# steineggerlab/Metabuli

Hardware: AMD Instinct MI355X
Metric: Mreads/s classified (metabuli classify hot path, reads + index resident in HBM) (higher is better)
Workload: dtype u64

## Files before the change

metabuli_amd/csrc/kernels_extract.h:

```cpp
#ifndef MTB_KERNELS_EXTRACT_H
#define MTB_KERNELS_EXTRACT_H
#include "dev_util.h"
#include "mtb_core.h"

#define MTB_EXTRACT_STAGE 320

struct ExtractArgs {
    const char *bases; const uint64_t *offs;
    const char *bases2; const uint64_t *offs2;
    uint64_t n_reads;
    int32_t seq_mode, syncmer, smer_len, kmer_format;
    int32_t tag_ord;
    int32_t dig_shift;
};

#define MTB_EXTRACT_BUF 320
#define MTB_EXTRACT_CHUNK 8192
template <int MODE>
__global__ __launch_bounds__(64) void k_extract(ExtractArgs a, const mtb_tables *__restrict__ tabs,
                                                uint32_t *__restrict__ counts, const uint64_t *__restrict__ out_offs,
                                                mtb_kmer *__restrict__ out, int32_t *__restrict__ qlen,
                                                int32_t *__restrict__ qlen2, uint32_t *__restrict__ max_len,
                                                unsigned long long *__restrict__ counter, uint64_t out_cap,
                                                uint16_t *__restrict__ dig_out = nullptr, uint8_t *__restrict__ off_flags = nullptr) {
    constexpr bool EMIT = MODE != 0;
    constexpr bool STATS = MODE != 1;
    __shared__ mtb_kmer s_out[MODE == 2 ? MTB_EXTRACT_BUF : 1];
    __shared__ unsigned long long s_base;
    uint32_t n_buf = 0;
    uint64_t chunk_pos = 0, chunk_end = 0, produced = 0, reads_done = 0, cur_read = 0;
    bool overflow = false;
    auto flush = [&]() {
        if (MODE != 2 || n_buf == 0) return;
        __syncthreads();
        uint32_t done = 0;
        while (done < n_buf) {
            if (chunk_pos == chunk_end) {
                const uint64_t need = n_buf - done;
                const uint64_t rem_reads = (a.n_reads - 1 - cur_read) / gridDim.x + 1;
                const uint64_t avg = reads_done ? produced / reads_done + 1 : 128;
                uint64_t size = need + rem_reads * avg * 5 / 4 + 64;
                size = size < MTB_EXTRACT_CHUNK ? size : MTB_EXTRACT_CHUNK;
                size = size < need ? need : size;
                if (threadIdx.x == 0) s_base = atomicAdd(counter, (unsigned long long)size);
                __syncthreads();
                chunk_pos = (uint64_t)s_base; chunk_end = chunk_pos + size;
                __syncthreads();
                if (chunk_end > out_cap) { overflow = true; chunk_pos = chunk_end; break; }
            }
            const uint32_t room = (uint32_t)(chunk_end - chunk_pos < (uint64_t)(n_buf - done) ? chunk_end - chunk_pos : (uint64_t)(n_buf - done));
            for (uint32_t i = threadIdx.x; i < room; i += 64) {
                const mtb_kmer x = s_out[done + i];
                out[chunk_pos + i] = x;
                if (dig_out) {
                    uint32_t two = (uint32_t)(x.value >> a.dig_shift) & 1023u, d = (two >> 5) * 21u + (two & 31u);
                    dig_out[chunk_pos + i] = (uint16_t)(d < 511u ? d : 511u);
                }
            }
            chunk_pos += room; done += room;
        }
        produced += n_buf;
        __syncthreads();
        n_buf = 0;
    };
    __shared__ mtb_tables s_tab;
    __shared__ __attribute__((aligned(8))) uint8_t s_cod[80];
    __shared__ __attribute__((aligned(8))) uint8_t s_cod3[MODE == 2 ? 3 : 1][MODE == 2 ? 120 : 8];
    __shared__ uint8_t s_code[MTB_EXTRACT_STAGE];
    const uint32_t lane = threadIdx.x;
    for (uint32_t i = lane; i < sizeof(mtb_tables) / 4; i += 64) ((uint32_t *)&s_tab)[i] = ((const uint32_t *)tabs)[i];
    __syncthreads();
    uint32_t my_max = 0, my_maxq = 0;
    uint32_t el_max = 0, el_maxq = 0, n_off = 0;
    const bool paired = a.seq_mode == 2;
    for (uint64_t r = blockIdx.x; r < a.n_reads; r += gridDim.x) {
        cur_read = r; reads_done++;
        const uint64_t o1 = a.offs[r];
        const int32_t len1 = (int32_t)(a.offs[r + 1] - o1);
        uint64_t o2 = 0; int32_t len2 = 0;
        if (paired) { o2 = a.offs2[r]; len2 = (int32_t)(a.offs2[r + 1] - o2); }
        const int32_t ql1 = mtb_used_len(len1), ql2 = paired ? mtb_used_len(len2) : 0;
        if (STATS) {
            if (lane == 0) { qlen[r] = ql1; qlen2[r] = ql2; }
            uint32_t tot_len = (uint32_t)(ql1 + ql2);
            my_max = tot_len > my_max ? tot_len : my_max;
        }
        const bool skip = mtb_read_too_short(len1) || (paired && mtb_read_too_short(len2));
        if (skip) { if ((MODE == 0 || (MODE == 2 && counts)) && lane == 0) counts[r] = 0; continue; }
        uint64_t wpos = MODE == 1 ? out_offs[r] : 0;
        uint32_t total = 0;
        for (int mate = 0; mate < (paired ? 2 : 1); mate++) {
            const char *seq = mate ? a.bases2 + o2 : a.bases + o1;
            const int32_t len = mate ? len2 : len1;
            const uint32_t pos_off = mate ? (uint32_t)(ql1 + 3) : 0u;
            const int32_t used = mtb_used_len(len);
            const int32_t n_cod = used / 3, n_win = n_cod - 7;
            const bool old_fmt = a.kmer_format == 1;
            const bool staged = !old_fmt && len <= MTB_EXTRACT_STAGE;
            if (staged) {
                __syncthreads();
                for (int32_t i = (int32_t)lane; i < len; i += 64) s_code[i] = s_tab.base[(uint8_t)seq[i]];
                __syncthreads();
            }
            if (MODE == 2 && staged) {
                for (int strand = 0; strand < 2; strand++) {
                    const bool fwd = strand == 0;
                    const bool back = !fwd;
                    __syncthreads();
                    for (int fi = 0; fi < 3; fi++) {
                        const int32_t begin = mtb_frame_begin(len, strand * 3 + fi);
                        for (int32_t j = (int32_t)lane; j < n_cod; j += 64)
                            s_cod3[fi][j] = mtb_codon_byte_codes(&s_tab, s_code, mtb_codon_ci(begin, used, j, fwd), fwd);
                    }
                    __syncthreads();
                    const int32_t n_all = 3 * n_win;
                    for (int32_t c0 = 0; c0 < n_all; c0 += 64) {
                        const int32_t cidx = c0 + (int32_t)lane;
                        const int32_t fi = (cidx >= n_win) + (cidx >= 2 * n_win);
                        const int32_t wi = cidx - fi * n_win;
                        const int32_t w = back ? n_win - 1 - wi : wi;
                        bool ok = false; uint64_t v = 0;
                        if (cidx < n_all) {
                            const uint32_t *c32 = (const uint32_t *)&s_cod3[fi][0];
                            const uint32_t q = (uint32_t)w >> 2, sh = (uint32_t)w & 3u;
                            const uint32_t x0 = c32[q], x1 = c32[q + 1], x2 = c32[q + 2];
                            ok = mtb_window_metamer_words(__builtin_amdgcn_alignbyte(x1, x0, sh), __builtin_amdgcn_alignbyte(x2, x1, sh), a.syncmer, a.smer_len, &v);
                        }
                        const uint64_t mask = __ballot(ok);
                        const uint32_t c = (uint32_t)__popcll(mask);
                        if (n_buf + c > MTB_EXTRACT_BUF) flush();
                        if (ok) {
                            const int f = strand * 3 + fi;
                            const int32_t begin = mtb_frame_begin(len, f);
                            const uint32_t below = (uint32_t)__popcll(mask & lanemask_lt());
                            uint32_t pf = mtb_window_pos(begin, used, w, fwd) + pos_off;
                            if (a.tag_ord) { const uint32_t ord = total + below; pf |= (ord < 0xFFFFu ? ord : 0xFFFFu) << 16; }
                            mtb_kmer k; k.value = v; k.qinfo = mtb_qinfo((uint32_t)(r + 1), pf, (uint32_t)f);
                            s_out[n_buf + below] = k;
                        }
                        n_buf += c; total += c;
                    }
                }
            } else
            for (int f = 0; f < 6; f++) {
                const bool fwd = f < 3;
                const int32_t begin = mtb_frame_begin(len, f);
                const bool back = MODE == 2 && a.tag_ord && (old_fmt ? fwd : !fwd);
                const int32_t n_chunk = (n_win + 63) / 64;
                for (int32_t cw = 0; cw < n_chunk; cw++) {
                    const int32_t w0 = (back ? n_chunk - 1 - cw : cw) * 64;
                    int32_t j = w0 + (int32_t)lane;
                    int32_t j2 = w0 + 64 + (int32_t)lane;
                    if (staged) {
                        if (j < n_cod) s_cod[lane] = mtb_codon_byte_codes(&s_tab, s_code, mtb_codon_ci(begin, used, j, fwd), fwd);
                        if (lane < 8 && j2 < n_cod) s_cod[64 + lane] = mtb_codon_byte_codes(&s_tab, s_code, mtb_codon_ci(begin, used, j2, fwd), fwd);
                    } else if (old_fmt) {
                        if (j < n_cod) s_cod[lane] = mtb_codon_byte_old(&s_tab, seq, mtb_codon_ci_old(begin, used, j, fwd), fwd);
                        if (lane < 8 && j2 < n_cod) s_cod[64 + lane] = mtb_codon_byte_old(&s_tab, seq, mtb_codon_ci_old(begin, used, j2, fwd), fwd);
                    } else {
                        if (j < n_cod) s_cod[lane] = mtb_codon_byte(&s_tab, seq, mtb_codon_ci(begin, used, j, fwd), fwd);
                        if (lane < 8 && j2 < n_cod) s_cod[64 + lane] = mtb_codon_byte(&s_tab, seq, mtb_codon_ci(begin, used, j2, fwd), fwd);
                    }
                    __syncthreads();
                    int32_t w = w0 + (int32_t)lane;
                    bool ok = false; uint64_t v = 0;
                    if (w < n_win) {
                        if (old_fmt) ok = mtb_window_metamer_old(&s_cod[lane], &v);
                        else {
                            const uint32_t *c32 = (const uint32_t *)s_cod;
                            const uint32_t q = lane >> 2, sh = lane & 3u;
                            const uint32_t x0 = c32[q], x1 = c32[q + 1], x2 = c32[q + 2];
                            ok = mtb_window_metamer_words(__builtin_amdgcn_alignbyte(x1, x0, sh), __builtin_amdgcn_alignbyte(x2, x1, sh), a.syncmer, a.smer_len, &v);
                        }
                    }
                    uint64_t mask = __ballot(ok);
                    uint32_t c = (uint32_t)__popcll(mask);
// ... 43 lines not shown
```

metabuli_amd/csrc/kernels_score_fast.h:

```cpp
#ifndef MTB_KERNELS_SCORE_FAST_H
#define MTB_KERNELS_SCORE_FAST_H
#include "dev_util.h"
#include "kernels_score.h"
#include "mtb_core.h"
#include "mtb_score_par.h"

#define MTB_FAST_BKT 128
#ifndef MTB_FAST_MERGE_SINGLES
#define MTB_FAST_MERGE_SINGLES 0
#endif

#ifdef MTB_FAST_DEBUG
__device__ unsigned long long mtb_fast_reasons[32];
#define MTB_FAST_COUNT(k, v) do { if (threadIdx.x == 0) atomicAdd(&mtb_fast_reasons[k], (unsigned long long)(v)); } while (0)
#define MTB_FAST_T0() unsigned long long ft_ = __builtin_readcyclecounter()
#define MTB_FAST_MARK(k) do { const unsigned long long t_ = __builtin_readcyclecounter(); if (threadIdx.x == 0) s_ph[k] += t_ - ft_; ft_ = t_; } while (0)
#else
#define MTB_FAST_COUNT(k, v) do {} while (0)
#define MTB_FAST_T0() do {} while (0)
#define MTB_FAST_MARK(k) do {} while (0)
#endif

#define MTB_DPP_RED(v, OP) do { \
    { const uint32_t o_ = (uint32_t)__builtin_amdgcn_update_dpp((int)(v), (int)(v), 0x111, 0xF, 0xF, false); (v) = OP((v), o_); } \
    { const uint32_t o_ = (uint32_t)__builtin_amdgcn_update_dpp((int)(v), (int)(v), 0x112, 0xF, 0xF, false); (v) = OP((v), o_); } \
    { const uint32_t o_ = (uint32_t)__builtin_amdgcn_update_dpp((int)(v), (int)(v), 0x114, 0xF, 0xF, false); (v) = OP((v), o_); } \
    { const uint32_t o_ = (uint32_t)__builtin_amdgcn_update_dpp((int)(v), (int)(v), 0x118, 0xF, 0xF, false); (v) = OP((v), o_); } \
    { const uint32_t o_ = (uint32_t)__builtin_amdgcn_update_dpp((int)(v), (int)(v), 0x142, 0xA, 0xF, false); (v) = OP((v), o_); } \
    { const uint32_t o_ = (uint32_t)__builtin_amdgcn_update_dpp((int)(v), (int)(v), 0x143, 0xC, 0xF, false); (v) = OP((v), o_); } } while (0)
#define MTB_MINU(a, b) ((b) < (a) ? (b) : (a))
#define MTB_MAXU(a, b) ((b) > (a) ? (b) : (a))
__device__ __forceinline__ uint32_t wave_min_u32(uint32_t v) { MTB_DPP_RED(v, MTB_MINU); return (uint32_t)__builtin_amdgcn_readlane((int)v, 63); }
__device__ __forceinline__ uint32_t wave_max_u32(uint32_t v) { MTB_DPP_RED(v, MTB_MAXU); return (uint32_t)__builtin_amdgcn_readlane((int)v, 63); }

struct FKey { uint32_t lo, hi; };
__device__ __forceinline__ uint32_t fk_species(const FKey &k) { return k.hi >> 10; }
__device__ __forceinline__ uint32_t fk_frame(const FKey &k) { return (k.hi >> 7) & 7u; }
__device__ __forceinline__ uint32_t fk_pos(const FKey &k) { return ((k.hi & 127u) << 4) | (k.lo >> 27); }
__device__ __forceinline__ uint32_t fk_ham(const FKey &k) { return (k.lo >> 24) & 7u; }
__device__ __forceinline__ uint32_t fk_dna(const FKey &k) { return k.lo & 0xFFFFFFu; }

struct FastPath { int32_t start, end; float score; int32_t ham; uint32_t rehs;  int32_t species; };

template <int K, int KL = K, bool BYFRAME = false>
__global__ __launch_bounds__(64, K <= 3 ? 5 : 4) void k_score_fast(const mtb_slot16 *__restrict__ slots_all, uint64_t n_reads, const int32_t *__restrict__ qlen,
                                                       const int32_t *__restrict__ qlen2, mtb_tax_view tx, mtb_score_params sp,
                                                       const uint64_t *__restrict__ tc_off, mtb_result *__restrict__ results,
                                                       int32_t *__restrict__ tc_tax, uint32_t *__restrict__ tc_cnt, uint64_t tc_cap, uint64_t tc_base,
                                                       const uint32_t *__restrict__ cursor, uint32_t stride, uint32_t direct, uint32_t epoch,
                                                       uint8_t *__restrict__ slow_flag, uint32_t *__restrict__ cnt_out) {
    constexpr int NMAX = 64 * K;
    __shared__ FKey s_key[NMAX];
    __shared__ uint64_t s_aux[NMAX];
    __shared__ uint64_t s_pp[NMAX];
    __shared__ FastPath s_path[64];
    __shared__ uint32_t s_pf[64];
    __shared__ uint32_t s_tl[(BYFRAME || MTB_FAST_MERGE_SINGLES) ? 64 : 1];
    typedef uint32_t __attribute__((may_alias)) u32a; typedef int32_t __attribute__((may_alias)) i32a;
    static_assert(NMAX * 8 >= 2 * MTB_FAST_BKT * 4 && NMAX * 8 >= 256 * 4 && NMAX * 8 >= (MTB_LR_MAXE + MTB_LR_MAXE * MTB_LR_K) * 4, "tables fit the arrays they live in");
    u32a *const s_hcnt = (u32a *)s_pp;
    u32a *const s_hmin = (u32a *)s_key; i32a *const s_btax = (i32a *)s_key + MTB_FAST_BKT;
    i32a *const s_otax = (i32a *)s_pp; u32a *const s_ocnt = (u32a *)s_pp + MTB_FAST_BKT;
    i32a *const s_lev = (i32a *)s_aux; i32a *const s_anc = (i32a *)s_aux + MTB_LR_MAXE;
    const int32_t lane = (int32_t)threadIdx.x;
    MTB_BEGIN_ACQUIRE();
#ifdef MTB_FAST_DEBUG
    __shared__ unsigned long long s_ph[16];
    if (threadIdx.x < 16) s_ph[threadIdx.x] = 0;
#endif
    const uint64_t lt = lanemask_lt();
    const uint64_t le = lt | (1ull << lane);
    const uint32_t tail_cap = stride - direct;
    const uint32_t div_m = (65536u + (uint32_t)sp.dna_shift - 1u) / (uint32_t)sp.dna_shift;
    const uint32_t lines = (stride * (uint32_t)sizeof(mtb_slot16) + 127u) / 128u;

    for (uint64_t r = blockIdx.x; r < n_reads; r += gridDim.x) {
        if (r + gridDim.x < n_reads && (uint32_t)lane < lines) {
            const uint8_t *pf = (const uint8_t *)(slots_all + (r + gridDim.x) * (uint64_t)stride) + (uint64_t)lane * 128u;
            __builtin_amdgcn_global_load_lds((const __attribute__((address_space(1))) void *)pf, (__attribute__((address_space(3))) void *)s_pf, 4, 0, 0);
        }
        MTB_FAST_T0();
        const int32_t ql1 = qlen[r], ql2 = qlen2[r];
        const int32_t read_len = ql1 + ql2;
        const int32_t nb = mtb_num_buckets(read_len, sp.dna_shift);
        const uint32_t cur = cursor[r];
        const mtb_slot16 *slots = slots_all + r * (uint64_t)stride;
        mtb_slot16 x[KL];
#pragma unroll
        for (int k = 0; k < KL; k++) { const uint32_t i = (uint32_t)lane + 64u * k; x[k].a = 0; x[k].b = 0; if (i < stride) x[k] = slots[i]; }
        bool slow = cur > tail_cap || nb > MTB_FAST_BKT;
        wave_fence();
        MTB_FAST_MARK(0);
        int32_t n = 0, n_live = 0;
        uint32_t spc[KL]; bool live[KL]; int32_t dst[KL];
        uint32_t smin = 0xFFFFFFFFu, smax = 0u;
#pragma unroll
        for (int k = 0; k < KL; k++) {
            const uint32_t i = (uint32_t)lane + 64u * k;
            live[k] = i < stride && mtb_slot_epoch(x[k]) == epoch && (i < direct || i - direct < cur);
            spc[k] = live[k] ? (uint32_t)(x[k].a >> 32) : 0xFFFFFFFFu;
            dst[k] = 0;
            n_live += (int32_t)__popcll(__ballot(live[k]));
            smin = spc[k] < smin ? spc[k] : smin;
            if (live[k]) smax = spc[k] > smax ? spc[k] : smax;
        }
        smin = wave_min_u32(smin); smax = wave_max_u32(smax);
        uint32_t todo_min = 0xFFFFFFFFu;
        if (smin != smax) {
            for (int32_t q = lane; q < 256; q += 64) s_hcnt[q] = 0;
            wave_fence();
#pragma unroll
            for (int k = 0; k < KL; k++) if (live[k]) atomicAdd(&s_hcnt[(spc[k] * 0x9E3779B1u) >> 24], 1u);
            wave_fence();
#pragma unroll
            for (int k = 0; k < KL; k++) if (live[k] && s_hcnt[(spc[k] * 0x9E3779B1u) >> 24] < 2u) { live[k] = false; spc[k] = 0xFFFFFFFFu; }
        } else if (n_live < 2) {
#pragma unroll
            for (int k = 0; k < KL; k++) { live[k] = false; spc[k] = 0xFFFFFFFFu; }
        }
        if (BYFRAME) {
#pragma unroll
            for (int k = 0; k < KL; k++) if (live[k]) spc[k] = (spc[k] << 3) | ((uint32_t)(x[k].b >> 52) & 7u);
        }
#pragma unroll
        for (int k = 0; k < KL; k++) todo_min = spc[k] < todo_min ? spc[k] : todo_min;
        for (int round = 0; ; round++) {
            const uint32_t m = wave_min_u32(todo_min);
            if (m == 0xFFFFFFFFu) break;
            if (round == 24) { slow = true; break; }
            todo_min = 0xFFFFFFFFu;
#pragma unroll
            for (int k = 0; k < KL; k++) {
                const bool mine = spc[k] == m;
                const uint64_t mask = __ballot(mine);
                if (mine) { dst[k] = n + (int32_t)__popcll(mask & lt); spc[k] = 0xFFFFFFFFu; }
                n += (int32_t)__popcll(mask);
                todo_min = spc[k] < todo_min ? spc[k] : todo_min;
            }
        }
        if (KL > K && n > NMAX) slow = true;
#pragma unroll
        for (int k = 0; k < KL; k++) {
            if (live[k] && !slow) {
                const uint64_t b = x[k].b;
                const uint32_t bh = (uint32_t)(b >> 32), ps_ = (bh >> 8) & 0x7FFu;
                FKey fk; fk.hi = ((uint32_t)(x[k].a >> 32) << 10) | (((bh >> 20) & 7u) << 7) | (ps_ >> 4);
                fk.lo = ((ps_ & 15u) << 27) | (((bh >> 23) & 7u) << 24) | ((uint32_t)b & 0xFFFFFFu);
                s_key[dst[k]] = fk;
                s_aux[dst[k]] = (x[k].a & 0xFFFFFFFFull) | (((b >> 24) & 0xFFFFull) << 32) | ((uint32_t)lane + 64u * k >= direct ? (1ull << 63) : 0ull);
            }
        }
        MTB_FAST_MARK(1);
        mtb_result R = mtb_result_blank(ql1, ql2, (uint32_t)tc_base);
        if (!slow && n == 0) { if (lane == 0) { cnt_out[r] = (uint32_t)n_live; results[r] = R; } continue; }
        wave_fence();
        {
            uint32_t nt = 0;
            bool any_tail = false;
#pragma unroll
            for (int k = 0; k < KL; k++) any_tail |= live[k] && (uint32_t)lane + 64u * k >= direct;
            if ((BYFRAME || MTB_FAST_MERGE_SINGLES) && !slow && __any(any_tail)) {
                FKey ke[K]; uint64_t ax[K]; int32_t np[K]; bool tl[K];
                const int32_t nsl = (n + 63) >> 6;
#pragma unroll
                for (int k = 0; k < K; k++) {
                    const int32_t i = lane + 64 * k;
                    ke[k].lo = 0; ke[k].hi = 0; ax[k] = 0; np[k] = i; tl[k] = false;
                    if (k < nsl && i < n) { ke[k] = s_key[i]; ax[k] = s_aux[i]; tl[k] = (ax[k] >> 63) != 0; }
                    if (k < nsl) {
                        const uint64_t tm = __ballot(tl[k]);
                        if (tl[k]) { const uint32_t at = nt + (uint32_t)__popcll(tm & lt); if (at < 64u) s_tl[at] = (uint32_t)i; }
                        nt += (uint32_t)__popcll(tm);
                    }
                }
                if (nt > 64u) slow = true;
                wave_fence();
                if (!slow) {
                    auto same_run = [&](const FKey &a, const FKey &b) { return BYFRAME ? ((a.hi ^ b.hi) >> 7) == 0 : ((a.hi ^ b.hi) >> 10) == 0; };
                    auto less = [&](const FKey &a, const FKey &b) { return a.hi < b.hi || (a.hi == b.hi && a.lo < b.lo); };
                    for (uint32_t t = 0; t < nt; t++) {
                        const int32_t ti = (int32_t)s_tl[t];
                        const FKey kt = s_key[ti];
                        uint32_t n_dir_less = 0, n_dir_run = 0;
#pragma unroll
                        for (int k = 0; k < K; k++) {
                            if (k < nsl) {
                                const int32_t i = lane + 64 * k;
                                const bool dir = i < n && !tl[k] && same_run(ke[k], kt);
                                const bool smaller = dir && less(ke[k], kt);
                                if (dir && !smaller) np[k]++;
                                n_dir_run += (uint32_t)__popcll(__ballot(dir)); n_dir_less += (uint32_t)__popcll(__ballot(smaller));
                            }
                        }
                        uint32_t n_tl_less = 0, n_tl_before = 0;
                        for (uint32_t u = 0; u < nt; u++) {
                            if (u == t) continue;
                            const FKey ku = s_key[s_tl[u]];
                            if (!same_run(ku, kt)) continue;
                            n_tl_less += (less(ku, kt) || (!less(kt, ku) && u < t)) ? 1u : 0u; n_tl_before += u < t ? 1u : 0u;
                        }
                        const int32_t run_start = ti - (int32_t)n_dir_run - (int32_t)n_tl_before;
#pragma unroll
                        for (int k = 0; k < K; k++) if (lane + 64 * k == ti) np[k] = run_start + (int32_t)(n_dir_less + n_tl_less);
                    }
                    wave_fence();
#pragma unroll
                    for (int k = 0; k < K; k++) { const int32_t i = lane + 64 * k; if (k < nsl && i < n) { s_key[np[k]] = ke[k]; s_aux[np[k]] = ax[k] & ~(1ull << 63); } }
                    wave_fence();
                }
            }
        }
        FKey key[K]; uint32_t tid[K], reh[K];
        int32_t tcanon[K]; uint8_t euk[K];
        const mtb_tax_node *nodes = (const mtb_tax_node *)tx.node;
        bool bhead[K], linked[K];
        int32_t shv[K];
        uint64_t bmask[K + 1], lmask[K + 1], rmask[K];
        const int32_t nslot = (n + 63) >> 6;
        bool bad = false, bad2 = false;
#ifdef MTB_FAST_DEBUG
        if (slow) MTB_FAST_COUNT(cur > tail_cap || nb > MTB_FAST_BKT ? 0 : 1, 1);
#endif
#pragma unroll
        for (int k = 0; k < K; k++) {
            const int32_t i = lane + 64 * k;
            key[k].lo = 0; key[k].hi = 0; tid[k] = 0; reh[k] = 0; bhead[k] = true; linked[k] = false; shv[k] = 0; tcanon[k] = -1; euk[k] = 0;
            bmask[k] = ~0ull; lmask[k] = 0; rmask[k] = 0;
            if (k < nslot && !slow) {
                FKey pk; pk.lo = 0; pk.hi = 0;
                if (i < n) {
                    key[k] = s_key[i]; const uint64_t a = s_aux[i]; tid[k] = (uint32_t)a; reh[k] = (uint32_t)(a >> 32) & 0xFFFFu; if (i > 0) pk = s_key[i - 1];
                }
                {
                    const int32_t t_ = (int32_t)tid[k], s_ = (int32_t)fk_species(key[k]);
                    const bool tv = i < n && t_ >= 0 && t_ <= tx.max_taxid, sv = i < n && s_ >= 0 && s_ <= tx.max_taxid;
                    const int32_t tc_ = nodes[tv ? t_ : 0].canon; const uint8_t eu_ = tx.under_euk[sv ? s_ : 0];
                    tcanon[k] = tv ? tc_ : -1; euk[k] = sv ? eu_ : 0;
                }
                const bool first = i == 0;
                if (i < n && !first) {
                    if (pk.hi > key[k].hi || (pk.hi == key[k].hi && pk.lo > key[k].lo)) bad = true;
                    if (pk.hi == key[k].hi && ((pk.lo ^ key[k].lo) >> 27) == 0) bad2 = true;
                }
                bhead[k] = i >= n || first || ((pk.hi ^ key[k].hi) >> 7) != 0;
                if (i < n && !bhead[k]) {
                    const int32_t pos = (int32_t)fk_pos(key[k]), ppos = (int32_t)fk_pos(pk);
                    const int32_t s = (pos - ppos) / 3;
                    if (s > 0 && s <= sp.max_codon_shift) {
                        shv[k] = s;
                        const bool fwd = fk_frame(key[k]) < 3u;
                        linked[k] = mtb_consecutive(fk_dna(pk), fk_dna(key[k]), s, fwd, sp.kmer_format);
                    }
                }
                bmask[k] = __ballot(bhead[k]);
                lmask[k] = __ballot(linked[k]);
                rmask[k] = __ballot(i < n && !linked[k]);
            }
        }
        bmask[K] = ~0ull; lmask[K] = 0;
#ifdef MTB_FAST_DEBUG
        if (!slow) { if (__any(bad)) MTB_FAST_COUNT(2, 1); else if (__any(bad2)) MTB_FAST_COUNT(3, 1); }
#endif
        slow = slow || __any(bad || bad2);
        if (slow) { if (lane == 0) slow_flag[r] = cur > tail_cap ? 2 : 1; continue; }
        if (lane == 0) cnt_out[r] = (uint32_t)n_live;
        MTB_FAST_MARK(2);
        float ps[K]; int32_t phd[K]; int32_t root[K];
        bool cand[K];
        {
            float carry_s = 0.0f; int32_t carry_hd = 0, last_root = 0;
#pragma unroll
            for (int k = 0; k < K; k++) {
                ps[k] = 0.0f; phd[k] = 0; root[k] = 0; cand[k] = false;
                if (k < nslot) {
                    const int32_t i = lane + 64 * k;
                    float is = 0.0f; int32_t ihd = 0;
                    if (linked[k]) mtb_link_inc(reh[k], shv[k], &is, &ihd);
                    ps[k] = wave_inclusive_scan_dpp(is) + carry_s; phd[k] = wave_inclusive_scan_dpp(ihd) + carry_hd;
                    carry_s = rl_f(ps[k], 63); carry_hd = rl_i(phd[k], 63);
                    const uint64_t mr = rmask[k];
                    const uint64_t lo_roots = mr & le;
                    root[k] = lo_roots ? 64 * k + 63 - (int32_t)__builtin_clzll(lo_roots) : last_root;
                    if (mr) last_root = 64 * k + 63 - (int32_t)__builtin_clzll(mr);
                    if (i < n) s_pp[i] = (uint64_t)__float_as_uint(ps[k]) | ((uint64_t)(uint32_t)phd[k] << 32);
                    const uint64_t bnext = (bmask[k] >> 1) | ((bmask[k + 1] & 1ull) << 63);
                    const uint64_t lnext = (lmask[k] >> 1) | ((lmask[k + 1] & 1ull) << 63);
                    const bool has_next = !((bnext >> lane) & 1ull);
                    const bool conn = (lnext >> lane) & 1ull;
                    cand[k] = i < n && (!bhead[k] || has_next) && !conn;
                }
            }
        }
        wave_fence();
        MTB_FAST_MARK(3);
        int32_t ne = 0;
        bool too_many = false;
#pragma unroll
        for (int k = 0; k < K; k++) {
            if (k < nslot) {
                bool e = false;
                FastPath P; P.start = 0; P.end = 0; P.score = 0.0f; P.ham = 0; P.rehs = 0; P.species = 0;
                if (cand[k]) {
                    const int32_t spc = (int32_t)fk_species(key[k]);
                    const int32_t md = euk[k] ? sp.min_cons_cnt_euk : sp.min_cons_cnt;
                    const int32_t rt = root[k];
                    const uint64_t pr = s_pp[rt]; const FKey rkey = s_key[rt];
                    const uint32_t rreh = (uint32_t)(s_aux[rt] >> 32);
                    const int32_t dhd = phd[k] - (int32_t)(uint32_t)(pr >> 32);
                    const int32_t depth = 1 + mtb_link_depth(dhd);
                    if (depth >= md) {
                        e = true;
                        P.start = (int32_t)fk_pos(rkey);
                        P.end = (int32_t)fk_pos(key[k]) + 23;
                        P.score = mtb_part_score(rreh, 8, false) + (rt == lane + 64 * k ? 0.0f : ps[k] - __uint_as_float((uint32_t)pr));
                        P.ham = (int32_t)fk_ham(rkey) + (rt == lane + 64 * k ? 0 : mtb_link_ham(dhd));
                        P.rehs = rreh | (reh[k] << 16);
                        P.species = spc;
// ... 170 lines not shown
```

metabuli_amd/csrc/mtb_api.hip:

```cpp
#include <hip/hip_runtime.h>

#include <fcntl.h>
#include <sys/stat.h>
#include <unistd.h>

#include <atomic>
#include <chrono>
#include <condition_variable>
#include <mutex>
#include <functional>
#include <map>
#include <string>
#include <thread>
#include <vector>

#include "../../include/mtb.h"
#include "host_db.h"
#include "host/merge_plan.h"
#include "host/audit_plan.h"
#include "kernels_extract.h"
#include "kernels_extract_blocks.h"
#include "kernels_index.h"
#include "kernels_join.h"
#include "kernels_build.h"
// ... 901 lines not shown
    hipLaunchKernelGGL(k_taxcnt_bound, dim3((uint32_t)((n_reads + 63) / 64)), dim3(64), 0, c->stream, d_seg, d_cnt, lens.d_ql, lens.d_ql2, n_reads, dna_shift, d_bound);
    { KTimer kt(c, MTB_K_SCAN); scan_launch<uint32_t, uint64_t, false>(c->stream, d_bound, n_reads, true, d_tcoff, d_ws); }
    STCHK(d2h(c, n_tc, d_tcoff + n_reads, 8));
    if (*n_tc > out.tc_cap) return fail(MTB_ERR_CAPACITY, "taxcnt buffers too small");
    if (out.tc_base + *n_tc >= (1ull << 32)) return fail(MTB_ERR_ARG, "more than 2^32-1 taxcnt slots in one batch (mtb_result.taxcnt_off is 32 bits); split the batch");
    return MTB_OK;
}
static mtb_status dev_score(mtb_ctx *c, mtb_index *ix, const mtb_params *p, uint64_t n_reads, const ReadLens &lens, const ResultSink &out, uint64_t *n_tc,
                            const ScoreSrc &first, const ScoreSecond *second) {
    mtb_score_params sp; mtb_make_score_params(p, &sp);
    uint64_t *d_tcoff;
    STCHK(ensure(c, "tcoff", n_reads + 1, &d_tcoff));
    STCHK(taxcnt_layout(c, n_reads, first.seg, first.cursor ? first.cursor : (const uint32_t *)first.bound_by_buckets, lens, out, sp.dna_shift, d_tcoff, n_tc));
    const bool key64 = ix->tax.max_id < (1 << 22) && lens.max_len + 3 < (1u << 11);
    const uint32_t max_nb_first = (uint32_t)mtb_num_buckets((int32_t)lens.max_len, sp.dna_shift);
    const uint32_t max_nb_second = (uint32_t)mtb_num_buckets((int32_t)std::max(lens.max_len, first.max_len_deferred), sp.dna_shift);
    if (max_nb_second > 65535u) return fail(MTB_ERR_ARG, "read too long for mtb_result.n_taxcnt (16 bits): more than 65535 position buckets");
    ScoreSrc second_src;
    for (int pass = 0; pass < 2; pass++) {
        const uint32_t max_nb = pass ? max_nb_second : max_nb_first;
        const ScoreSrc *S = &first;
        if (pass == 1) {
            if (!second) break;
            bool go = false;
            const ScoreLaunch SL{d_tcoff, key64, sp, lens, out};
            STCHK((*second)(&second_src, &go, SL));
            if (!go) break;
            S = &second_src;
        }
        uint32_t grid = S->grid ? S->grid : (uint32_t)std::min<uint64_t>(n_reads, std::max<uint64_t>(256ull * 14, n_reads / 8));
        bool need_slab = S->max_seg > S->cap || max_nb > MTB_SCORE_BKT;
        uint32_t slab_n = need_slab ? std::max<uint32_t>(S->max_seg, 1) : 0;
        uint32_t slab_nb = need_slab ? max_nb : 0;
        uint64_t slab_bytes = need_slab ? score_slab_bytes(slab_n, slab_nb) : 0;
        uint8_t *d_slabs = nullptr;
        const bool dynamic = need_slab && !S->cursor;
        if (dynamic) grid = std::min<uint32_t>(grid, 256u * 14u);
        if (slab_bytes) {
            while ((uint64_t)grid * slab_bytes > (MTB_SLAB_POOL_MAX) && grid > 64) grid /= 2;
            STCHK(ensure(c, "slabs", (size_t)grid * slab_bytes, &d_slabs, BUF_FIXED));
        }
        unsigned long long *d_work = nullptr;
        if (dynamic) { d_work = scal<unsigned long long>(c, SC_SCORE_WORK) + pass; HIPCHK(hipMemsetAsync(d_work, 0, 8, c->stream)); }
#define MTB_LAUNCH_SCORE(SRT, K, CAPV, DYNV, SLOTV) hipLaunchKernelGGL((k_score<SRT, K, mtb_match, CAPV, DYNV, SLOTV>), dim3(grid), dim3(64), 0, c->stream, S->m, S->seg, n_reads, lens.d_ql, \
        lens.d_ql2, tax_view(ix), sp, (const uint64_t *)d_tcoff, out.d_res, out.d_tc_tax, out.d_tc_cnt, out.tc_cap, d_slabs, slab_bytes, slab_n, slab_nb, (mtb_match *)nullptr,  \
        out.tc_base, S->list, S->n_list, S->cursor, S->stride, S->seg_by_list, S->direct, S->epoch, S->big_list, S->n_big, S->cnt_out, d_work, S->only_flagged, S->seg_cnt)
        ScoreSrc S_rest;
        const bool pairs = p->seq_mode == 2;
        if (S->cursor && pass == 0 && key64 && S->stride <= 384u && !c->opt.no_fast_scorer && !(pairs && c->opt.no_fast_pairs)) {
            uint8_t *d_slow;
            STCHK(ensure(c, "slowflag", n_reads, &d_slow));
            HIPCHK(hipMemsetAsync(d_slow, 0, n_reads, c->stream));
            HIPCHK(scal_clear(c, SC_N_GENERIC));
#define MTB_LAUNCH_FAST(...) hipLaunchKernelGGL((k_score_fast<__VA_ARGS__>), dim3(grid), dim3(64), 0, c->stream, (const mtb_slot16 *)S->m, n_reads, lens.d_ql, lens.d_ql2, tax_view(ix), sp, \
            (const uint64_t *)d_tcoff, out.d_res, out.d_tc_tax, out.d_tc_cnt, out.tc_cap, out.tc_base, S->cursor, S->stride, S->direct, S->epoch, d_slow, S->cnt_out)
            { KTimer ktf(c, MTB_K_SCORE_FAST);
              if (pairs) { if (S->stride <= 192) MTB_LAUNCH_FAST(3, 3, true); else if (S->stride <= 256) MTB_LAUNCH_FAST(4, 4, true); else MTB_LAUNCH_FAST(5, 6, true); }
              else if (S->stride <= 128) MTB_LAUNCH_FAST(2); else if (S->stride <= 192) MTB_LAUNCH_FAST(3); else if (S->stride <= 256) MTB_LAUNCH_FAST(4); else MTB_LAUNCH_FAST(5, 6, false); }
#undef MTB_LAUNCH_FAST
            hipLaunchKernelGGL(k_count_flags, dim3(256), dim3(256), 0, c->stream, (const uint8_t *)d_slow, n_reads, scal<unsigned long long>(c, SC_N_GENERIC));
            if (S->big_list && S->n_big) hipLaunchKernelGGL(k_list_flag2, dim3((uint32_t)((n_reads + 255) / 256)), dim3(256), 0, c->stream, (const uint8_t *)d_slow, n_reads, S->big_list, S->n_big);
            c->fast_used = true;
            S_rest = *S; S_rest.only_flagged = d_slow;
            S = &S_rest;
        }
        KTimer kt(c, pass == 0 ? MTB_K_SCORE : MTB_K_SEGSORT);
        if (S->cursor) {
#define MTB_LAUNCH_SLOT(CAPV) do { if (key64) MTB_LAUNCH_SCORE(true, true, CAPV, false, true); else MTB_LAUNCH_SCORE(true, false, CAPV, false, true); } while (0)
            if (S->cap <= 144) MTB_LAUNCH_SLOT(144);
            else if (S->cap <= 160) MTB_LAUNCH_SLOT(160);
            else if (S->cap <= 224) MTB_LAUNCH_SLOT(224);
            else if (S->cap <= 288) MTB_LAUNCH_SLOT(288);
            else MTB_LAUNCH_SLOT(320);
#undef MTB_LAUNCH_SLOT
        } else if (dynamic) {
            if (!S->sort) MTB_LAUNCH_SCORE(false, false, MTB_SCORE_LDS, true, false);
            else if (key64) MTB_LAUNCH_SCORE(true, true, MTB_SCORE_LDS, true, false); else MTB_LAUNCH_SCORE(true, false, MTB_SCORE_LDS, true, false);
        }
        else if (S->sort) { if (key64) MTB_LAUNCH_SCORE(true, true, MTB_SCORE_LDS, false, false); else MTB_LAUNCH_SCORE(true, false, MTB_SCORE_LDS, false, false); }
        else if (S->cap >= 320) MTB_LAUNCH_SCORE(false, false, 320, false, false);
        else MTB_LAUNCH_SCORE(false, false, MTB_SCORE_LDS, false, false);
#undef MTB_LAUNCH_SCORE
    }
    HIPCHK(hipGetLastError());
    return MTB_OK;
}

struct LongSegs {
    const mtb_match *d_m = nullptr; const uint64_t *d_seg = nullptr; uint32_t max_seg = 0;
    const uint32_t *d_segcnt = nullptr, *d_list = nullptr; uint32_t n_list = 0;
};
static mtb_status dev_score_long(mtb_ctx *c, mtb_index *ix, const mtb_params *p, uint64_t n_reads, const ReadLens &lens, const ResultSink &out, uint64_t *n_tc, const LongSegs &sg) {
    mtb_score_params sp; mtb_make_score_params(p, &sp);
    uint64_t *d_tcoff; uint8_t *d_todo;
    STCHK(ensure(c, "tcoff", n_reads + 1, &d_tcoff)); STCHK(ensure(c, "slowflag", n_reads, &d_todo));
    if (!sg.d_list) {
        STCHK(taxcnt_layout(c, n_reads, sg.d_seg, sg.d_segcnt, lens, out, sp.dna_shift, d_tcoff, n_tc));
        const uint32_t max_nb = (uint32_t)mtb_num_buckets((int32_t)lens.max_len, sp.dna_shift);
        if (max_nb > 65535u) return fail(MTB_ERR_ARG, "read too long for mtb_result.n_taxcnt (16 bits): more than 65535 position buckets");
    }
    HIPCHK(hipMemsetAsync(d_todo, 0, n_reads, c->stream));
    unsigned long long *d_work = scal<unsigned long long>(c, SC_LONG_WORK);
    HIPCHK(hipMemsetAsync(d_work, 0, 8, c->stream));
    HIPCHK(scal_clear(c, SC_LONG_N_SECOND));
    {   KTimer kt(c, MTB_K_SCORE_FAST);
        const uint64_t n_it = sg.d_list ? sg.n_list : n_reads;
        hipLaunchKernelGGL((k_score_long<MTB_LONG_MAXBLK, MTB_LONG_MAXSP, 512, 2048>), dim3((uint32_t)std::min<uint64_t>(n_it, 256ull * 4)), dim3(MTB_LONG_NT), 0, c->stream, sg.d_m, sg.d_seg, n_reads, lens.d_ql, lens.d_ql2, tax_view(ix), sp, (const uint64_t *)d_tcoff,
                           out.d_res, out.d_tc_tax, out.d_tc_cnt, out.tc_cap, out.tc_base, d_todo, d_work, sg.d_segcnt, sg.d_list, sg.n_list, 0u);
        hipLaunchKernelGGL(k_count_flags, dim3(256), dim3(256), 0, c->stream, (const uint8_t *)d_todo, n_reads, scal<unsigned long long>(c, SC_LONG_N_SECOND));
        uint64_t n_second = 0;
        STCHK(d2h(c, &n_second, scal<uint64_t>(c, SC_LONG_N_SECOND), 8));
// ... 2934 lines not shown
```

metabuli_amd/csrc/mtb_core.h:

```cpp
#ifndef MTB_CORE_H
#define MTB_CORE_H
#include <stdint.h>
#include "../../include/mtb.h"

#if defined(__HIPCC__)
#define MTB_HD __host__ __device__ __forceinline__
#else
#define MTB_HD inline
#endif
#if defined(__HIPCC__)
#define MTB_UNROLL _Pragma("unroll")
#else
#define MTB_UNROLL
#endif

MTB_HD uint64_t mtb_qinfo(uint32_t seq_id, uint32_t pos, uint32_t frame) {
    return (uint64_t)pos | ((uint64_t)(seq_id & 0x1FFFFFFFu) << 32) | ((uint64_t)(frame & 7u) << 61);
}
MTB_HD uint32_t mtb_q_pos(uint64_t q)   { return (uint32_t)q; }
MTB_HD uint32_t mtb_q_seq(uint64_t q)   { return (uint32_t)((q >> 32) & 0x1FFFFFFFu); }
MTB_HD uint32_t mtb_q_frame(uint64_t q) { return (uint32_t)(q >> 61); }

MTB_HD int32_t mtb_used_len(int32_t len) {
    int32_t r = len % 3;
// ... 24 lines not shown
    for (int i = 0; i < 64; i++) {
        char r = AA_ACTG[i];
        int aa = 20;
        if (r != '*') { aa = 0; while (LET[aa] != r) aa++; }
        int cid = i & 3;
        t->codon[i] = (uint8_t)(aa | (cid << 5));
    }
    #define MTB_SETCID(c0, c1, c2, id) t->codon[(c0) * 16 + (c1) * 4 + (c2)] = (uint8_t)((t->codon[(c0) * 16 + (c1) * 4 + (c2)] & 31) | ((id) << 5))
    MTB_SETCID(0, 3, 3, 4); MTB_SETCID(0, 3, 0, 5);
    MTB_SETCID(2, 2, 3, 4); MTB_SETCID(2, 2, 0, 5);
    MTB_SETCID(0, 3, 2, 6); MTB_SETCID(0, 3, 1, 7);
    MTB_SETCID(2, 3, 0, 5);
    #undef MTB_SETCID
    static const uint8_t H[8][8] = {
        {0, 1, 1, 1, 2, 1, 3, 3}, {1, 0, 1, 1, 2, 2, 3, 2},
        {1, 1, 0, 1, 2, 2, 2, 3}, {1, 1, 1, 0, 1, 2, 3, 3},
        {2, 2, 2, 1, 0, 1, 4, 4}, {1, 2, 2, 2, 1, 0, 4, 4},
        {3, 3, 2, 3, 4, 4, 0, 1}, {3, 2, 3, 3, 4, 4, 1, 0}};
    for (int a = 0; a < 8; a++) {
        uint32_t w = 0;
        for (int b = 0; b < 8; b++) w |= (uint32_t)H[a][b] << (4 * b);
        t->hamrow[a] = w;
    }
}

MTB_HD uint8_t mtb_codon_byte_old(const mtb_tables *t, const char *seq, int64_t ci, bool fwd) {
    uint32_t a, b, c;
    if (fwd) { a = t->base[(uint8_t)seq[ci - 2]]; b = t->base[(uint8_t)seq[ci - 1]]; c = t->base[(uint8_t)seq[ci]]; }
    else {
        a = t->base[(uint8_t)seq[ci + 2]]; b = t->base[(uint8_t)seq[ci + 1]]; c = t->base[(uint8_t)seq[ci]];
        if ((a | b | c) < 4) { a ^= 2; b ^= 2; c ^= 2; }
    }
    if ((a | b | c) > 3) return 0xFF;
    return t->codon[a * 16 + b * 4 + c];
}
MTB_HD uint8_t mtb_codon_byte(const mtb_tables *t, const char *seq, int64_t ci, bool fwd) {
    uint32_t a, b, c;
    if (fwd) {
        a = t->base[(uint8_t)seq[ci]]; b = t->base[(uint8_t)seq[ci + 1]]; c = t->base[(uint8_t)seq[ci + 2]];
    } else {
        a = t->base[(uint8_t)seq[ci]]; b = t->base[(uint8_t)seq[ci - 1]]; c = t->base[(uint8_t)seq[ci - 2]];
        if ((a | b | c) < 4) { a ^= 2; b ^= 2; c ^= 2; }
    }
    if ((a | b | c) > 3) return 0xFF;
    return t->codon[a * 16 + b * 4 + c];
}

MTB_HD uint8_t mtb_codon_byte_codes(const mtb_tables *t, const uint8_t *code, int64_t ci, bool fwd) {
    uint32_t a, b, c;
    if (fwd) { a = code[ci]; b = code[ci + 1]; c = code[ci + 2]; }
    else { a = code[ci]; b = code[ci - 1]; c = code[ci - 2]; if ((a | b | c) < 4) { a ^= 2; b ^= 2; c ^= 2; } }
    if ((a | b | c) > 3) return 0xFF;
    return t->codon[a * 16 + b * 4 + c];
}

MTB_HD int32_t mtb_frame_begin(int32_t len, int32_t frame) {
    if (frame < 3) return frame;
    int32_t b = (len % 3) - (frame % 3);
    return b < 0 ? b + 3 : b;
}
MTB_HD int64_t mtb_codon_ci(int32_t begin, int32_t used, int32_t j, bool fwd) {
    return fwd ? (int64_t)begin + 3 * (int64_t)j : (int64_t)begin + used - 1 - 3 * (int64_t)j;
}
MTB_HD int64_t mtb_codon_ci_old(int32_t begin, int32_t used, int32_t j, bool fwd) {
    return fwd ? (int64_t)begin + used - 1 - 3 * (int64_t)j : (int64_t)begin + 3 * (int64_t)j;
}
MTB_HD uint32_t mtb_window_pos_old(int32_t begin, int32_t used, int32_t p, bool fwd) {
    return fwd ? (uint32_t)(begin + used - 1 - (p + 8) * 3 + 1) : (uint32_t)(begin + 3 * p);
}
MTB_HD uint32_t mtb_window_pos(int32_t begin, int32_t used, int32_t p, bool fwd) {
    return fwd ? (uint32_t)(begin + 3 * p) : (uint32_t)(begin + used - 1 - (p + 8) * 3 + 1);
}

MTB_HD bool mtb_window_metamer_old(const uint8_t *cod, uint64_t *value) {
    uint64_t aa = 0, dna = 0;
    uint32_t bad = 0;
MTB_UNROLL
    for (int i = 0; i < 8; i++) {
        uint32_t b = cod[i];
        bad |= (b == 0xFFu);
        aa = aa * 21u + (b & 31u);
        dna = (dna << 3) | (b >> 5);
    }
    if (bad) return false;
    *value = (aa << 24) | (dna & 0xFFFFFFull);
    return true;
}
MTB_HD uint32_t mtb_pack_aa4(uint32_t w) {
    uint32_t x = ((w & 0x001F001Fu) << 5) | ((w >> 8) & 0x001F001Fu);
    return ((x & 0x3FFu) << 10) | (x >> 16);
}
MTB_HD uint32_t mtb_pack_cid4(uint32_t w) {
    uint32_t y = (w >> 5) & 0x07070707u;
    uint32_t p = ((y & 0x00070007u) << 3) | ((y >> 8) & 0x00070007u);
    return ((p & 0x3Fu) << 6) | (p >> 16);
}
MTB_HD bool mtb_window_metamer_words(uint32_t w0, uint32_t w1, int syncmer, int smer_len, uint64_t *value) {
    uint32_t bad = (((w0 & 0x1F1F1F1Fu) + 0x01010101u) | ((w1 & 0x1F1F1F1Fu) + 0x01010101u)) & 0x20202020u;
    if (bad) return false;
    const uint32_t a0 = mtb_pack_aa4(w0), a1 = mtb_pack_aa4(w1);
    const uint32_t dna = (mtb_pack_cid4(w0) << 12) | mtb_pack_cid4(w1);
    const uint64_t aa = ((uint64_t)a0 << 20) | a1;
    *value = (aa << 24) | dna;
    if (!syncmer) return true;
    if (smer_len == 5) {
        const uint32_t s0 = (a0 << 5) | (a1 >> 15), s1 = ((a0 & 0x7FFFu) << 10) | (a1 >> 10);
// ... 585 lines not shown
```

Baseline: 70.63.

## Share codon translation across strands and add tail-merge repair for single-end fast scoring

The extract kernel now translates each codon window once, producing forward and reverse-complement codes from the same five bases, and fills all six frames in one pass with one barrier. Before, each strand and frame reloaded and translated codons separately. The fast scorer gains a REPAIR template path, enabled by default for single-end reads. When the sort check fails and tail entries exist, it runs the tail merge and retries, so fewer reads go to the slow path. The tail-merge inner loop is now done with lane shuffles and ballots instead of a serial loop over shared memory, and oversized reads exit before their slots are loaded.

Result: slower. 69.09 (-2.2%).

```diff
diff --git a/metabuli_amd/csrc/kernels_extract.h b/metabuli_amd/csrc/kernels_extract.h
--- a/metabuli_amd/csrc/kernels_extract.h
+++ b/metabuli_amd/csrc/kernels_extract.h
@@ -65,7 +65,7 @@
     };
     __shared__ mtb_tables s_tab;
     __shared__ __attribute__((aligned(8))) uint8_t s_cod[80];
-    __shared__ __attribute__((aligned(8))) uint8_t s_cod3[MODE == 2 ? 3 : 1][MODE == 2 ? 120 : 8];
+    __shared__ __attribute__((aligned(8))) uint8_t s_cod3[MODE == 2 ? 6 : 1][MODE == 2 ? 120 : 8];
     __shared__ uint8_t s_code[MTB_EXTRACT_STAGE];
     const uint32_t lane = threadIdx.x;
     for (uint32_t i = lane; i < sizeof(mtb_tables) / 4; i += 64) ((uint32_t *)&s_tab)[i] = ((const uint32_t *)tabs)[i];
@@ -103,16 +103,22 @@
                 __syncthreads();
             }
             if (MODE == 2 && staged) {
+                {
+                    const int32_t lm = len % 3;
+                    for (int32_t j = (int32_t)lane; j < n_cod; j += 64) {
+                        uint8_t fw[3], rv[3];
+                        mtb_codon_bytes_both(&s_tab, s_code, j, fw, rv);
+#pragma unroll
+                        for (int b = 0; b < 3; b++) {
+                            s_cod3[b][j] = fw[b];
+                            s_cod3[3 + (lm + 3 - b) % 3][n_cod - 1 - j] = rv[b];
+                        }
+                    }
+                    __syncthreads();
+                }
                 for (int strand = 0; strand < 2; strand++) {
                     const bool fwd = strand == 0;
                     const bool back = !fwd;
-                    __syncthreads();
-                    for (int fi = 0; fi < 3; fi++) {
-                        const int32_t begin = mtb_frame_begin(len, strand * 3 + fi);
-                        for (int32_t j = (int32_t)lane; j < n_cod; j += 64)
-                            s_cod3[fi][j] = mtb_codon_byte_codes(&s_tab, s_code, mtb_codon_ci(begin, used, j, fwd), fwd);
-                    }
-                    __syncthreads();
                     const int32_t n_all = 3 * n_win;
                     for (int32_t c0 = 0; c0 < n_all; c0 += 64) {
                         const int32_t cidx = c0 + (int32_t)lane;
@@ -121,7 +127,7 @@
                         const int32_t w = back ? n_win - 1 - wi : wi;
                         bool ok = false; uint64_t v = 0;
                         if (cidx < n_all) {
-                            const uint32_t *c32 = (const uint32_t *)&s_cod3[fi][0];
+                            const uint32_t *c32 = (const uint32_t *)&s_cod3[strand * 3 + fi][0];
                             const uint32_t q = (uint32_t)w >> 2, sh = (uint32_t)w & 3u;
                             const uint32_t x0 = c32[q], x1 = c32[q + 1], x2 = c32[q + 2];
                             ok = mtb_window_metamer_words(__builtin_amdgcn_alignbyte(x1, x0, sh), __builtin_amdgcn_alignbyte(x2, x1, sh), a.syncmer, a.smer_len, &v);
diff --git a/metabuli_amd/csrc/kernels_score_fast.h b/metabuli_amd/csrc/kernels_score_fast.h
--- a/metabuli_amd/csrc/kernels_score_fast.h
+++ b/metabuli_amd/csrc/kernels_score_fast.h
@@ -6,9 +6,6 @@
 #include "mtb_score_par.h"
 
 #define MTB_FAST_BKT 128
-#ifndef MTB_FAST_MERGE_SINGLES
-#define MTB_FAST_MERGE_SINGLES 0
-#endif
 
 #ifdef MTB_FAST_DEBUG
 __device__ unsigned long long mtb_fast_reasons[32];
@@ -42,7 +39,7 @@
 
 struct FastPath { int32_t start, end; float score; int32_t ham; uint32_t rehs;  int32_t species; };
 
-template <int K, int KL = K, bool BYFRAME = false>
+template <int K, int KL = K, bool BYFRAME = false, bool REPAIR = false>
 __global__ __launch_bounds__(64, K <= 3 ? 5 : 4) void k_score_fast(const mtb_slot16 *__restrict__ slots_all, uint64_t n_reads, const int32_t *__restrict__ qlen,
                                                        const int32_t *__restrict__ qlen2, mtb_tax_view tx, mtb_score_params sp,
                                                        const uint64_t *__restrict__ tc_off, mtb_result *__restrict__ results,
@@ -55,7 +52,7 @@
     __shared__ uint64_t s_pp[NMAX];
     __shared__ FastPath s_path[64];
     __shared__ uint32_t s_pf[64];
-    __shared__ uint32_t s_tl[(BYFRAME || MTB_FAST_MERGE_SINGLES) ? 64 : 1];
+    __shared__ uint32_t s_tl[(BYFRAME || REPAIR) ? 64 : 1];
     typedef uint32_t __attribute__((may_alias)) u32a; typedef int32_t __attribute__((may_alias)) i32a;
     static_assert(NMAX * 8 >= 2 * MTB_FAST_BKT * 4 && NMAX * 8 >= 256 * 4 && NMAX * 8 >= (MTB_LR_MAXE + MTB_LR_MAXE * MTB_LR_K) * 4, "tables fit the arrays they live in");
     u32a *const s_hcnt = (u32a *)s_pp;
@@ -84,11 +81,12 @@
         const int32_t read_len = ql1 + ql2;
         const int32_t nb = mtb_num_buckets(read_len, sp.dna_shift);
         const uint32_t cur = cursor[r];
+        if (cur > tail_cap || nb > MTB_FAST_BKT) { MTB_FAST_COUNT(0, 1); if (lane == 0) slow_flag[r] = cur > tail_cap ? 2 : 1; continue; }
         const mtb_slot16 *slots = slots_all + r * (uint64_t)stride;
         mtb_slot16 x[KL];
 #pragma unroll
         for (int k = 0; k < KL; k++) { const uint32_t i = (uint32_t)lane + 64u * k; x[k].a = 0; x[k].b = 0; if (i < stride) x[k] = slots[i]; }
-        bool slow = cur > tail_cap || nb > MTB_FAST_BKT;
+        bool slow = false;
         wave_fence();
         MTB_FAST_MARK(0);
         int32_t n = 0, n_live = 0;
@@ -154,12 +152,13 @@
         mtb_result R = mtb_result_blank(ql1, ql2, (uint32_t)tc_base);
         if (!slow && n == 0) { if (lane == 0) { cnt_out[r] = (uint32_t)n_live; results[r] = R; } continue; }
         wave_fence();
-        {
+        bool any_tail = false;
+#pragma unroll
+        for (int k = 0; k < KL; k++) any_tail |= live[k] && (uint32_t)lane + 64u * k >= direct;
+        const bool has_tail = (BYFRAME || REPAIR) && __any(any_tail);
+        auto tail_merge = [&]() {
             uint32_t nt = 0;
-            bool any_tail = false;
-#pragma unroll
-            for (int k = 0; k < KL; k++) any_tail |= live[k] && (uint32_t)lane + 64u * k >= direct;
-            if ((BYFRAME || MTB_FAST_MERGE_SINGLES) && !slow && __any(any_tail)) {
+            {
                 FKey ke[K]; uint64_t ax[K]; int32_t np[K]; bool tl[K];
                 const int32_t nsl = (n + 63) >> 6;
 #pragma unroll
@@ -178,9 +177,11 @@
                 if (!slow) {
                     auto same_run = [&](const FKey &a, const FKey &b) { return BYFRAME ? ((a.hi ^ b.hi) >> 7) == 0 : ((a.hi ^ b.hi) >> 10) == 0; };
                     auto less = [&](const FKey &a, const FKey &b) { return a.hi < b.hi || (a.hi == b.hi && a.lo < b.lo); };
+                    FKey tk; tk.lo = 0; tk.hi = 0; int32_t tpos = 0;
+                    if ((uint32_t)lane < nt) { tpos = (int32_t)s_tl[lane]; tk = s_key[tpos]; }
                     for (uint32_t t = 0; t < nt; t++) {
-                        const int32_t ti = (int32_t)s_tl[t];
-                        const FKey kt = s_key[ti];
+                        const int32_t ti = rl_i(tpos, (int32_t)t);
+                        FKey kt; kt.lo = (uint32_t)rl_i((int32_t)tk.lo, (int32_t)t); kt.hi = (uint32_t)rl_i((int32_t)tk.hi, (int32_t)t);
                         uint32_t n_dir_less = 0, n_dir_run = 0;
 #pragma unroll
                         for (int k = 0; k < K; k++) {
@@ -192,13 +193,9 @@
                                 n_dir_run += (uint32_t)__popcll(__ballot(dir)); n_dir_less += (uint32_t)__popcll(__ballot(smaller));
                             }
                         }
-                        uint32_t n_tl_less = 0, n_tl_before = 0;
-                        for (uint32_t u = 0; u < nt; u++) {
-                            if (u == t) continue;
-                            const FKey ku = s_key[s_tl[u]];
-                            if (!same_run(ku, kt)) continue;
-                            n_tl_less += (less(ku, kt) || (!less(kt, ku) && u < t)) ? 1u : 0u; n_tl_before += u < t ? 1u : 0u;
-                        }
+                        const bool in_run = (uint32_t)lane < nt && (uint32_t)lane != t && same_run(tk, kt);
+                        const uint32_t n_tl_less = (uint32_t)__popcll(__ballot(in_run && (less(tk, kt) || (!less(kt, tk) && (uint32_t)lane < t))));
+                        const uint32_t n_tl_before = (uint32_t)__popcll(__ballot(in_run && (uint32_t)lane < t));
                         const int32_t run_start = ti - (int32_t)n_dir_run - (int32_t)n_tl_before;
 #pragma unroll
                         for (int k = 0; k < K; k++) if (lane + 64 * k == ti) np[k] = run_start + (int32_t)(n_dir_less + n_tl_less);
@@ -209,7 +206,8 @@
                     wave_fence();
                 }
             }
-        }
+        };
+        if (BYFRAME && !slow && has_tail) tail_merge();
         FKey key[K]; uint32_t tid[K], reh[K];
         int32_t tcanon[K]; uint8_t euk[K];
         const mtb_tax_node *nodes = (const mtb_tax_node *)tx.node;
@@ -219,50 +217,55 @@
         const int32_t nslot = (n + 63) >> 6;
         bool bad = false, bad2 = false;
 #ifdef MTB_FAST_DEBUG
-        if (slow) MTB_FAST_COUNT(cur > tail_cap || nb > MTB_FAST_BKT ? 0 : 1, 1);
-#endif
-#pragma unroll
-        for (int k = 0; k < K; k++) {
-            const int32_t i = lane + 64 * k;
-            key[k].lo = 0; key[k].hi = 0; tid[k] = 0; reh[k] = 0; bhead[k] = true; linked[k] = false; shv[k] = 0; tcanon[k] = -1; euk[k] = 0;
-            bmask[k] = ~0ull; lmask[k] = 0; rmask[k] = 0;
-            if (k < nslot && !slow) {
-                FKey pk; pk.lo = 0; pk.hi = 0;
-                if (i < n) {
-                    key[k] = s_key[i]; const uint64_t a = s_aux[i]; tid[k] = (uint32_t)a; reh[k] = (uint32_t)(a >> 32) & 0xFFFFu; if (i > 0) pk = s_key[i - 1];
-                }
-                {
-                    const int32_t t_ = (int32_t)tid[k], s_ = (int32_t)fk_species(key[k]);
-                    const bool tv = i < n && t_ >= 0 && t_ <= tx.max_taxid, sv = i < n && s_ >= 0 && s_ <= tx.max_taxid;
-                    const int32_t tc_ = nodes[tv ? t_ : 0].canon; const uint8_t eu_ = tx.under_euk[sv ? s_ : 0];
-                    tcanon[k] = tv ? tc_ : -1; euk[k] = sv ? eu_ : 0;
-                }
-                const bool first = i == 0;
-                if (i < n && !first) {
-                    if (pk.hi > key[k].hi || (pk.hi == key[k].hi && pk.lo > key[k].lo)) bad = true;
-                    if (pk.hi == key[k].hi && ((pk.lo ^ key[k].lo) >> 27) == 0) bad2 = true;
-                }
-                bhead[k] = i >= n || first || ((pk.hi ^ key[k].hi) >> 7) != 0;
-                if (i < n && !bhead[k]) {
-                    const int32_t pos = (int32_t)fk_pos(key[k]), ppos = (int32_t)fk_pos(pk);
-                    const int32_t s = (pos - ppos) / 3;
-                    if (s > 0 && s <= sp.max_codon_shift) {
-                        shv[k] = s;
-                        const bool fwd = fk_frame(key[k]) < 3u;
-                        linked[k] = mtb_consecutive(fk_dna(pk), fk_dna(key[k]), s, fwd, sp.kmer_format);
-                    }
-                }
-                bmask[k] = __ballot(bhead[k]);
-                lmask[k] = __ballot(linked[k]);
-                rmask[k] = __ballot(i < n && !linked[k]);
-            }
+        if (slow) MTB_FAST_COUNT(1, 1);
+#endif
+        for (int attempt = 0; ; attempt++) {
+            bad = false; bad2 = false;
+#pragma unroll
+            for (int k = 0; k < K; k++) {
+                const int32_t i = lane + 64 * k;
+                key[k].lo = 0; key[k].hi = 0; tid[k] = 0; reh[k] = 0; bhead[k] = true; linked[k] = false; shv[k] = 0; tcanon[k] = -1; euk[k] = 0;
+                bmask[k] = ~0ull; lmask[k] = 0; rmask[k] = 0;
+                if (k < nslot && !slow) {
+                    FKey pk; pk.lo = 0; pk.hi = 0;
+                    if (i < n) {
+                        key[k] = s_key[i]; const uint64_t a = s_aux[i]; tid[k] = (uint32_t)a; reh[k] = (uint32_t)(a >> 32) & 0xFFFFu; if (i > 0) pk = s_key[i - 1];
+                    }
+                    {
+                        const int32_t t_ = (int32_t)tid[k], s_ = (int32_t)fk_species(key[k]);
+                        const bool tv = i < n && t_ >= 0 && t_ <= tx.max_taxid, sv = i < n && s_ >= 0 && s_ <= tx.max_taxid;
+                        const int32_t tc_ = nodes[tv ? t_ : 0].canon; const uint8_t eu_ = tx.under_euk[sv ? s_ : 0];
+                        tcanon[k] = tv ? tc_ : -1; euk[k] = sv ? eu_ : 0;
+                    }
+                    const bool first = i == 0;
+                    if (i < n && !first) {
+                        if (pk.hi > key[k].hi || (pk.hi == key[k].hi && pk.lo > key[k].lo)) bad = true;
+                        if (pk.hi == key[k].hi && ((pk.lo ^ key[k].lo) >> 27) == 0) bad2 = true;
+                    }
+                    bhead[k] = i >= n || first || ((pk.hi ^ key[k].hi) >> 7) != 0;
+                    if (i < n && !bhead[k]) {
+                        const int32_t pos = (int32_t)fk_pos(key[k]), ppos = (int32_t)fk_pos(pk);
+                        const int32_t s = (pos - ppos) / 3;
+                        if (s > 0 && s <= sp.max_codon_shift) {
+                            shv[k] = s;
+                            const bool fwd = fk_frame(key[k]) < 3u;
+                            linked[k] = mtb_consecutive(fk_dna(pk), fk_dna(key[k]), s, fwd, sp.kmer_format);
+                        }
+                    }
+                    bmask[k] = __ballot(bhead[k]);
+                    lmask[k] = __ballot(linked[k]);
+                    rmask[k] = __ballot(i < n && !linked[k]);
+                }
+            }
+            if (!REPAIR || BYFRAME || attempt || slow || !has_tail || !__any(bad)) break;
+            tail_merge();
         }
         bmask[K] = ~0ull; lmask[K] = 0;
 #ifdef MTB_FAST_DEBUG
         if (!slow) { if (__any(bad)) MTB_FAST_COUNT(2, 1); else if (__any(bad2)) MTB_FAST_COUNT(3, 1); }
 #endif
         slow = slow || __any(bad || bad2);
-        if (slow) { if (lane == 0) slow_flag[r] = cur > tail_cap ? 2 : 1; continue; }
+        if (slow) { if (lane == 0) slow_flag[r] = 1; continue; }
         if (lane == 0) cnt_out[r] = (uint32_t)n_live;
         MTB_FAST_MARK(2);
         float ps[K]; int32_t phd[K]; int32_t root[K];
diff --git a/metabuli_amd/csrc/mtb_api.hip b/metabuli_amd/csrc/mtb_api.hip
--- a/metabuli_amd/csrc/mtb_api.hip
+++ b/metabuli_amd/csrc/mtb_api.hip
@@ -977,11 +977,15 @@
             STCHK(ensure(c, "slowflag", n_reads, &d_slow));
             HIPCHK(hipMemsetAsync(d_slow, 0, n_reads, c->stream));
             HIPCHK(scal_clear(c, SC_N_GENERIC));
+#ifndef MTB_FAST_REPAIR_S1
+#define MTB_FAST_REPAIR_S1 true
+#endif
 #define MTB_LAUNCH_FAST(...) hipLaunchKernelGGL((k_score_fast<__VA_ARGS__>), dim3(grid), dim3(64), 0, c->stream, (const mtb_slot16 *)S->m, n_reads, lens.d_ql, lens.d_ql2, tax_view(ix), sp, \
             (const uint64_t *)d_tcoff, out.d_res, out.d_tc_tax, out.d_tc_cnt, out.tc_cap, out.tc_base, S->cursor, S->stride, S->direct, S->epoch, d_slow, S->cnt_out)
             { KTimer ktf(c, MTB_K_SCORE_FAST);
               if (pairs) { if (S->stride <= 192) MTB_LAUNCH_FAST(3, 3, true); else if (S->stride <= 256) MTB_LAUNCH_FAST(4, 4, true); else MTB_LAUNCH_FAST(5, 6, true); }
-              else if (S->stride <= 128) MTB_LAUNCH_FAST(2); else if (S->stride <= 192) MTB_LAUNCH_FAST(3); else if (S->stride <= 256) MTB_LAUNCH_FAST(4); else MTB_LAUNCH_FAST(5, 6, false); }
+              else if (S->stride <= 128) MTB_LAUNCH_FAST(2, 2, false, MTB_FAST_REPAIR_S1); else if (S->stride <= 192) MTB_LAUNCH_FAST(3, 3, false, MTB_FAST_REPAIR_S1);
+              else if (S->stride <= 256) MTB_LAUNCH_FAST(4, 4, false, MTB_FAST_REPAIR_S1); else MTB_LAUNCH_FAST(5, 6, false, MTB_FAST_REPAIR_S1); }
 #undef MTB_LAUNCH_FAST
             hipLaunchKernelGGL(k_count_flags, dim3(256), dim3(256), 0, c->stream, (const uint8_t *)d_slow, n_reads, scal<unsigned long long>(c, SC_N_GENERIC));
             if (S->big_list && S->n_big) hipLaunchKernelGGL(k_list_flag2, dim3((uint32_t)((n_reads + 255) / 256)), dim3(256), 0, c->stream, (const uint8_t *)d_slow, n_reads, S->big_list, S->n_big);
diff --git a/metabuli_amd/csrc/mtb_core.h b/metabuli_amd/csrc/mtb_core.h
--- a/metabuli_amd/csrc/mtb_core.h
+++ b/metabuli_amd/csrc/mtb_core.h
@@ -100,6 +100,17 @@
     else { a = code[ci]; b = code[ci - 1]; c = code[ci - 2]; if ((a | b | c) < 4) { a ^= 2; b ^= 2; c ^= 2; } }
     if ((a | b | c) > 3) return 0xFF;
     return t->codon[a * 16 + b * 4 + c];
+}
+
+MTB_HD void mtb_codon_bytes_both(const mtb_tables *t, const uint8_t *code, int32_t j, uint8_t *fw, uint8_t *rv) {
+    uint32_t c[5];
+    for (int i = 0; i < 5; i++) c[i] = code[3 * j + i];
+    for (int b = 0; b < 3; b++) {
+        const bool ok = (c[b] | c[b + 1] | c[b + 2]) < 4;
+        const uint32_t f_ = (c[b] * 16 + c[b + 1] * 4 + c[b + 2]) & 63u, r_ = ((c[b + 2] * 16 + c[b + 1] * 4 + c[b]) ^ 0x2Au) & 63u;
+        fw[b] = ok ? t->codon[f_] : (uint8_t)0xFF;
+        rv[b] = ok ? t->codon[r_] : (uint8_t)0xFF;
+    }
 }
 
 MTB_HD int32_t mtb_frame_begin(int32_t len, int32_t frame) {
```
